# wmtlab/tactileSR

Hardware: AMD Instinct MI355X
Metric: SR samples/sec (4x4->40x40) (higher is better)
Workload: dtype f32 as 2 power-of-two-scaled fp16 planes x 3 MFMA products, fp32 accumulate (fp32-grade); 1 GPU; tactileSR_model eval forward 4x4->40x40, batch=4096/GPU, fp32 in/out (BASELINE configs[1]); batch_per_gpu=4096, scale_factor=10, seqsCnt=1, parallelism=replicas x1, conv_impl=fp16x3, dist_world_size=1

## Files before the change

### tactilesr_amd/csrc/conv_mfma_k32.hip

```cpp
#include "tsr_common.h"
#include "conv_args.h"
#include "conv_epilogue16.h"
#include "conv_fuse1x1_16.h"
#include "tactilesr_hip.h"
#include <type_traits>

typedef _Float16 kf16x8 __attribute__((ext_vector_type(8)));
typedef _Float16 kf16x4 __attribute__((ext_vector_type(4)));

constexpr int k32_row_slots(int px) {
  int rs = px * 4;
  while ((rs & 3) != 2) ++rs;
  return rs;
}

template <int KS, int COUT, int WN, bool DBH = false, int NTHR = 256> struct K32Geom {
  static constexpr int IMG = (NTHR / 64) / WN;
  static constexpr int HH = 8 + KS - 1;
  static constexpr int T = KS * KS;
  static constexpr int HS = (T - 1) / 2;
  static constexpr int PIXB = 64;
  static constexpr int ROWB = k32_row_slots(HH) * 16;
  static constexpr int IMGB = HH * ROWB;
  static constexpr int HALO_B = IMG * IMGB;
  static constexpr int SROWB = k32_row_slots(8) * 16;
  static constexpr int SIMGB = 8 * SROWB;
  static constexpr int SIDE_B = DBH ? 0 : IMG * SIMGB;
  static constexpr int WTAP_B = 2 * 16 * COUT * 2;
  static constexpr int WSLAB_B = 2 * WTAP_B;
  static constexpr int NHB = DBH ? 2 : 1;
  static constexpr int MAIN_LDS = NHB * HALO_B + SIDE_B + 3 * WSLAB_B;
};

constexpr int PAIR_KH[12] = {0, 0, 0, 2, 1, 3, 4, 4, 1, 1, 2, 3};
constexpr int PAIR_KW[12] = {0, 2, 4, 4, 0, 0, 1, 3, 1, 3, 1, 1};
constexpr int PAIR_V[12] = {0, 0, 1, 1, 1, 1, 0, 0, 0, 1, 0, 0};
constexpr int PAIR_OUTER = 8;

template <int KS, int COUT, bool EXT, int WN, bool FUSE2 = false, bool DBH = false, int NTHR = 256, bool PAIR = false>
__global__ __launch_bounds__(NTHR, NTHR == 512 ? 1 : 2) void conv_k32_kernel(const ConvArgs a) {
  static_assert(!PAIR || (KS == 5 && COUT == 128 && !EXT && !FUSE2 && !DBH), "pair form: 5x5 geometry, inference");
  static_assert(COUT == 64 * WN, "every wave owns 64 channels");
  static_assert(!FUSE2 || (!EXT && COUT == 128), "fused 1x1: 128 channels, inference");
  static_assert(NTHR == 256 || (NTHR == 512 && WN == 2), "512 threads: 4 images x 2 C_out halves");
  typedef K32Geom<KS, COUT, WN, DBH, NTHR> G;
  constexpr int NW = NTHR / 64;
  constexpr bool WDMA = !EXT;
  constexpr int IMG = G::IMG, P = KS / 2, HH = G::HH, T = G::T, HS = G::HS, NT = COUT / (16 * WN);
  constexpr int PIXB = G::PIXB, ROWB = G::ROWB, IMGB = G::IMGB, HALO_B = G::HALO_B;
  constexpr int SROWB = G::SROWB, SIMGB = G::SIMGB, SIDE_B = G::SIDE_B;
  constexpr int WTAP_B = G::WTAP_B, WSLAB_B = G::WSLAB_B;
  constexpr int WITEMS = WSLAB_B / 16, WV = (WITEMS + NTHR - 1) / NTHR;
  constexpr int NITEM = IMG * HH * HH * 4, NIT = (NITEM + NTHR - 1) / NTHR;
  constexpr int FUSE_LDS = FUSE2 ? Fuse1x1Geom16<IMG>::BYTES + 64 : 0;
  __shared__ __attribute__((aligned(16))) char lds[G::MAIN_LDS > FUSE_LDS ? G::MAIN_LDS : FUSE_LDS];
  char* halo = lds;
  char* wbuf = lds + G::NHB * HALO_B + SIDE_B;

  const int tid = threadIdx.x;
  const int lane = tid & 63;
  const int wave = tid >> 6;
  const int wave_s = __builtin_amdgcn_readfirstlane(wave);
  const int wm = WN == 2 ? wave >> 1 : wave, wn = WN == 2 ? wave & 1 : 0;
  const int m = lane & 15, g = lane >> 4, khalf = g & 1, tsel = g >> 1;

  float sx = 1.f, accmul = 1.f, sxh = 1.f;
  int bid;
  {
    const int nwg = gridDim.x, q = nwg >> 3, r = nwg & 7;
    const int xcd = blockIdx.x & 7, idx = blockIdx.x >> 3;
    bid = (xcd < r ? xcd * (q + 1) : r * (q + 1) + (xcd - r) * q) + idx;
  }
  const int tpi = a.tiles_x * a.tiles_y;
  const int ig = bid / tpi;
  const int trem = bid - ig * tpi;
  const int ebase = bid * IMG;
  const int ty = trem / a.tiles_x, tx = trem - ty * a.tiles_x;
  const int y0 = ty * 8, x0 = tx * 8, b0 = ig * IMG;
  const int HW = a.H * a.W;
  const int in_blocks = a.in_ctot >> 4;

  int st_src[NIT], st_dst[NIT];
#pragma unroll
  for (int k = 0; k < NIT; ++k) {
    const int it = tid + k * NTHR;
    st_src[k] = -1;
    st_dst[k] = -1;
    if (it < NITEM) {
      const int qd = it & 3, px = it >> 2;
      const int img = px / (HH * HH), rem = px - img * (HH * HH);
      const int hy = rem / HH, hx = rem - hy * HH;
      const int gy = y0 - P + hy, gx = x0 - P + hx, b = b0 + img;
      st_dst[k] = img * IMGB + hy * ROWB + hx * PIXB + qd * 8;
      if (b < a.B && gy >= 0 && gy < a.H && gx >= 0 && gx < a.W)
        st_src[k] = ((img * in_blocks) * HW + gy * a.W + gx) * 16 + qd * 4;
    }
  }
  const float* in_base = a.in + ((size_t)b0 * in_blocks + (a.in_coff >> 4)) * HW * 16;

  const int laneA0 = wm * IMGB + (m >> 3) * ROWB + (m & 7) * PIXB + khalf * 16;
  const int lx = laneA0 + tsel * PIXB;
  constexpr int CK = PAIR ? 3 : KS - 1;
  const int lw = PAIR ? laneA0 + tsel * ROWB
                      : laneA0 + tsel * (ROWB - (KS - 1) * PIXB);
  const int lc = tsel ? laneA0 + CK * ROWB + CK * PIXB
                      : HALO_B + wm * SIMGB + (m >> 3) * SROWB + (m & 7) * PIXB + khalf * 16;
  const int lcs = tsel ? 2 * ROWB : 2 * SROWB;
  const int lcd = laneA0 + (KS - 1) * (ROWB + PIXB) + tsel * HALO_B;
  const int laneB = tsel * WTAP_B + (khalf * COUT + wn * (COUT / WN) + m) * 16;
  const int laneBh = tsel * (WTAP_B / 2) + (khalf * 64 + wn * 32 + m) * 16;

  f32x4 acc[4][NT];
#pragma unroll
  for (int mt = 0; mt < 4; ++mt)
#pragma unroll
    for (int nt = 0; nt < NT; ++nt) acc[mt][nt] = (f32x4){0.f, 0.f, 0.f, 0.f};

  const int nreal = a.cin >> 4;
  const int nchunk = nreal + (nreal & 1);
  const int S = (nchunk >> 1) * T;
  const char* wsrc = (const char*)a.wp;
  const __amdgpu_buffer_rsrc_t wrsrc = __builtin_amdgcn_make_buffer_rsrc((void*)a.wp, 0, 0x7fffffff, 0x00020000);

  f32x4 hsc = {1.f, 1.f, 1.f, 1.f}, hsh = {0.f, 0.f, 0.f, 0.f};
  auto load_halo = [&](int c, f32x4* hv) __attribute__((always_inline)) {
    const float* inc = in_base + (size_t)(c < nreal ? c : nreal - 1) * HW * 16;
    if (EXT && a.in_scale) {
      const int cq = (c < nreal ? c : nreal - 1) * 16 + (tid & 3) * 4;
      hsc = *(const f32x4*)(a.in_scale + cq);
      hsh = *(const f32x4*)(a.in_shift + cq);
    }
#pragma unroll
    for (int k = 0; k < NIT; ++k) hv[k] = *(const f32x4*)(inc + (unsigned)(st_src[k] < 0 ? 0 : st_src[k]));
  };
  auto store_halo = [&](const f32x4* hv, int c, int hb = 0) __attribute__((always_inline)) {
#pragma unroll
    for (int k = 0; k < NIT; ++k) {
      if (st_dst[k] >= 0) {
        f32x4 v = hv[k];
        if (EXT && a.in_scale) {
#pragma unroll
          for (int jj = 0; jj < 4; ++jj) v[jj] = tsr_relu_x2(fmaf(v[jj], hsc[jj], hsh[jj]));
        }
        const bool inside = st_src[k] >= 0 && c < nreal;
#pragma unroll
        for (int jj = 0; jj < 4; ++jj) v[jj] = inside ? v[jj] * sxh : 0.f;
#pragma unroll
        for (int p = 0; p < 2; ++p) {
          kf16x4 bq;
#pragma unroll
          for (int jj = 0; jj < 4; ++jj) {
            bq[jj] = (_Float16)v[jj];
            v[jj] -= (float)bq[jj];
          }
          *(kf16x4*)(halo + hb * HALO_B + st_dst[k] + p * 32) = bq;
        }
      }
    }
  };
#define DMA_BYTES(goff_, slot_, nv_)                                                     \
  {                                                                                      \
    const int vo_ = (int)(goff_) + tid * 16;                                             \
    char* dst_ = wbuf + (slot_) * WSLAB_B + wave_s * 1024;                               \
    _Pragma("unroll") for (int v = 0; v < (nv_); ++v)                                    \
      __builtin_amdgcn_raw_ptr_buffer_load_lds(wrsrc, (__attribute__((address_space(3))) void*)(dst_ + v * NTHR * 16), 16, \
                                               vo_ + v * NTHR * 16, 0, 0, 0);             \
  }
#define LOAD_W(sidx)                                                                     \
  {                                                                                      \
    const f32x4* src_ = (const f32x4*)(wsrc + (size_t)(sidx) * WSLAB_B);                  \
    _Pragma("unroll") for (int v = 0; v < WV; ++v) wreg[v] = src_[tid + v * NTHR];        \
  }
#define STORE_W(slot)                                                                    \
  {                                                                                      \
    char* wb_ = wbuf + (slot) * WSLAB_B;                                                 \
    _Pragma("unroll") for (int v = 0; v < WV; ++v) ((f32x4*)wb_)[tid + v * NTHR] = wreg[v]; \
  }
#define DMA_W(sidx, slot) DMA_BYTES((size_t)(sidx) * WSLAB_B, slot, WV)
#define DMA_WAIT_N(n_) __builtin_amdgcn_s_waitcnt(0x0F70 | ((n_) & 15) | (((n_) >> 4) << 14))
#define DMA_WAIT() DMA_WAIT_N(0)
#define PAIR_HALF(pq_) ((pq_) < 24 && ((pq_) % 12) < PAIR_OUTER)
#define DMA_WP(slot, pq_)                                                                \
  {                                                                                      \
    if (PAIR_HALF(pq_)) { DMA_BYTES(woff, slot, WV / 2); woff += WSLAB_B / 2; }          \
    else { DMA_BYTES(woff, slot, WV); woff += WSLAB_B; }                                 \
  }
#define STEP_BARRIER() __syncthreads()
#define LOAD_A(dst, p_, st_, hb_)                                                        \
  {                                                                                      \
    const int kh_ = PAIR ? PAIR_KH[(st_)] : (2 * (st_)) / KS, kw_ = PAIR ? PAIR_KW[(st_)] : (2 * (st_)) - kh_ * KS; \
    const bool x_ = PAIR ? PAIR_V[(st_)] == 0 : kw_ < KS - 1;                            \
    const char* ab_ = lds + (x_ ? lx : lw) + (hb_) * HALO_B + kh_ * ROWB + kw_ * PIXB + (p_) * 32; \
    _Pragma("unroll") for (int mt = 0; mt < 4; ++mt) dst[mt] = *(const kf16x8*)(ab_ + mt * 2 * ROWB); \
  }
#define LOAD_A_CROSS(dst, p_)                                                            \
  {                                                                                      \
    _Pragma("unroll") for (int mt = 0; mt < 4; ++mt) dst[mt] = *(const kf16x8*)(lds + lc + mt * lcs + (p_) * 32); \
  }
#define LOAD_A_CROSSD(dst, p_)                                                           \
  {                                                                                      \
    _Pragma("unroll") for (int mt = 0; mt < 4; ++mt) dst[mt] = *(const kf16x8*)(lds + lcd + mt * 2 * ROWB + (p_) * 32); \
  }
#define LOAD_B(dst, p_, slot_)                                                           \
  {                                                                                      \
    const char* wb_ = wbuf + (slot_) * WSLAB_B + laneB + (p_) * (2 * COUT * 16);         \
    _Pragma("unroll") for (int nt = 0; nt < NT; ++nt) dst[nt] = *(const kf16x8*)(wb_ + nt * 256); \
  }
#define LOAD_B_HI(dst, p_, slot_)                                                        \
  {                                                                                      \
    const char* wb_ = wbuf + (slot_) * WSLAB_B + laneBh + (p_) * (2 * 64 * 16);          \
    _Pragma("unroll") for (int nt = 2; nt < NT; ++nt) dst[nt] = *(const kf16x8*)(wb_ + (nt - 2) * 256); \
  }
#define MFMA_PHASE_HI(A_, B_)                                                            \
  _Pragma("unroll") for (int mt = 0; mt < 4; ++mt)                                       \
    _Pragma("unroll") for (int nt = 2; nt < NT; ++nt)                                    \
      acc[mt][nt] = __builtin_amdgcn_mfma_f32_16x16x32_f16(A_[mt], B_[nt], acc[mt][nt], 0, 0, 0);
#define MFMA_PHASE(A_, B_)                                                               \
  _Pragma("unroll") for (int mt = 0; mt < 4; ++mt)                                       \
    _Pragma("unroll") for (int nt = 0; nt < NT; ++nt)                                    \
      acc[mt][nt] = __builtin_amdgcn_mfma_f32_16x16x32_f16(A_[mt], B_[nt], acc[mt][nt], 0, 0, 0);
#define INTERLEAVE(n_, per_)                                                             \
  _Pragma("unroll") for (int i_ = 0; i_ < (n_); ++i_) {                                  \
    __builtin_amdgcn_sched_group_barrier(0x008, (per_), 0);                              \
    __builtin_amdgcn_sched_group_barrier(0x100, 1, 0);                                   \
  }

  auto operand_scales = [&]() __attribute__((always_inline)) {
    float mx = a.in_amax ? *a.in_amax : 0.f;
    if (EXT && a.in_scale) {
      __shared__ float bnd[2 * NW];
      float ms = 0.f, mt = 0.f;
      for (int c = threadIdx.x; c < a.cin; c += NTHR) {
        ms = fmaxf(ms, fabsf(a.in_scale[c]));
        mt = fmaxf(mt, fabsf(a.in_shift[c]));
      }
#pragma unroll
      for (int o = 32; o > 0; o >>= 1) {
        ms = fmaxf(ms, __shfl_xor(ms, o));
        mt = fmaxf(mt, __shfl_xor(mt, o));
      }
      if (lane == 0) { bnd[wave * 2] = ms; bnd[wave * 2 + 1] = mt; }
      __syncthreads();
      ms = 0.f; mt = 0.f;
#pragma unroll
      for (int w = 0; w < NW; ++w) { ms = fmaxf(ms, bnd[2 * w]); mt = fmaxf(mt, bnd[2 * w + 1]); }
      mx = mx * ms + mt;
    }
    if (mx > 0.f) {
      int e = (int)((__float_as_uint(mx) >> 23) & 0xFF) - 127;
      int be = 13 - e + 127;
      be = be < 1 ? 1 : (be > 254 ? 254 : be);
      sx = __uint_as_float((unsigned)be << 23);
    }
    float w_inv = a.w_inv_scale;
    if (a.w_amax) {
      const float wmx = *a.w_amax;
      w_inv = 1.f;
      if (wmx > 0.f && wmx < 3.0e38f) {
        int be = 127 - (13 - ((int)((__float_as_uint(wmx) >> 23) & 0xFF) - 127));
        be = be < 1 ? 1 : (be > 254 ? 254 : be);
        w_inv = __uint_as_float((unsigned)be << 23);
      }
    }
    accmul = w_inv / sx;
    sxh = (EXT && a.in_scale) ? 0.5f * sx : sx;
  };

  f32x4 hv[NIT], wreg[WDMA ? 1 : WV];
  size_t woff = 0;
  load_halo(0, hv);
  if constexpr (PAIR) {
    DMA_WP(0, 0);
    DMA_WP(1, 1);
    operand_scales();
  } else if constexpr (WDMA) {
    DMA_W(0, 0);
    if (S > 1) DMA_W(1, 1);
    operand_scales();
  } else {
    LOAD_W(0);
    operand_scales();
    STORE_W(0);
    if (S > 1) { LOAD_W(1); STORE_W(1); }
  }
  store_halo(hv, 0);
  if constexpr (WDMA) { DMA_WAIT(); } else { if (S > 2) LOAD_W(2); }
  __syncthreads();

  kf16x8 A0[4], A1[4], B0[NT] = {}, B1[NT] = {};
  LOAD_A(A1, 1, 0, 0);
  if constexpr (PAIR) { LOAD_B_HI(B0, 0, 0); } else { LOAD_B(B0, 0, 0); }

  constexpr int SCI = IMG * 256 / NTHR, SCS = NTHR / 256;
  const int sc_t = tid & 255, sc_i0 = tid >> 8;
  const int sc_src = sc_i0 * IMGB + ((sc_t >> 5) + CK) * ROWB + (((sc_t >> 2) & 7) + CK) * PIXB + (sc_t & 3) * 16;
  const int sc_dst = HALO_B + sc_i0 * SIMGB + (sc_t >> 5) * SROWB + ((sc_t >> 2) & 7) * PIXB + (sc_t & 3) * 16;

  int s = 0;
  int slot = 0;
  auto block = [&](int c, auto oddc) __attribute__((always_inline)) {
    constexpr int ODD = decltype(oddc)::value;
    constexpr int NST = HS + ODD;
#pragma unroll
    for (int st = 0; st < NST; ++st) {
      const int slot1 = slot == 2 ? 0 : slot + 1;
      const int slot2 = slot1 == 2 ? 0 : slot1 + 1;
      const bool cross = ODD && st == HS;
      f32x4 sidev[SCI];
      if (WDMA && s + 2 < S) {
        if constexpr (PAIR) { DMA_WP(slot2, (ODD * HS + st + 2) % 25); } else { DMA_W(s + 2, slot2); }
      }
      const bool outer = PAIR && st < PAIR_OUTER;
      const bool next_outer = PAIR && (st + 1 < PAIR_OUTER || st + 1 == NST);
      if (cross) { LOAD_A_CROSS(A0, 0); } else { LOAD_A(A0, 0, st, 0); }
      if (outer) { LOAD_B_HI(B1, 1, slot); } else { LOAD_B(B1, 1, slot); }
      if (!ODD && st == 0) {
#pragma unroll
        for (int k = 0; k < SCI; ++k) sidev[k] = *(const f32x4*)(lds + sc_src + k * SCS * IMGB);
      }
      if (st == NST - 2 && c + 1 < nchunk) load_halo(c + 1, hv);
      if (outer) {
        MFMA_PHASE_HI(A1, B0);
        if (!ODD && st == 0) { INTERLEAVE(6 + SCI, 1); } else { INTERLEAVE(6, 1); }
      } else {
        MFMA_PHASE(A1, B0);
        if (!ODD && st == 0) { INTERLEAVE(8 + SCI, 1); } else { INTERLEAVE(8, 2); }
      }
      if (st + 1 < NST) {
        if (ODD && st + 1 == HS) { LOAD_A_CROSS(A1, 1); } else { LOAD_A(A1, 1, st + 1, 0); }
      }
      if (outer) {
        MFMA_PHASE_HI(A0, B0);
        if (st + 1 < NST) { INTERLEAVE(4, 2); }
      } else {
        MFMA_PHASE(A0, B0);
        if (st + 1 < NST) { INTERLEAVE(4, 4); }
      }
      if (next_outer) { LOAD_B_HI(B0, 0, slot1); } else { LOAD_B(B0, 0, slot1); }
      if (outer) {
        MFMA_PHASE_HI(A0, B1);
        if (next_outer) { INTERLEAVE(2, 4); } else { INTERLEAVE(4, 2); }
      } else {
        MFMA_PHASE(A0, B1);
        if (next_outer) { INTERLEAVE(2, 8); } else { INTERLEAVE(4, 4); }
      }
      if (!ODD && st == 0) {
#pragma unroll
        for (int k = 0; k < SCI; ++k) *(f32x4*)(lds + sc_dst + k * SCS * SIMGB) = sidev[k];
      }
      if constexpr (WDMA) {
        if (st == NST - 2 && c + 1 < nchunk) { DMA_WAIT_N(NIT); } else { DMA_WAIT(); }
      } else {
        if (s + 2 < S) STORE_W(slot2);
        if (s + 3 < S) LOAD_W(s + 3);
      }
      STEP_BARRIER();
      if (st + 1 == NST && c + 1 < nchunk) {
        store_halo(hv, c + 1);
        __syncthreads();
        LOAD_A(A1, 1, 0, 0);
      }
      ++s;
      slot = slot1;
    }
  };
  if constexpr (!DBH) {
    for (int c = 0; c < nchunk; c += 2) {
      block(c, std::integral_constant<int, 0>());
      block(c + 1, std::integral_constant<int, 1>());
    }
  } else {
    for (int c = 0; c < nchunk; c += 2) {
#pragma unroll
      for (int p = 0; p < T; ++p) {
        const int slot1 = slot == 2 ? 0 : slot + 1;
        const int slot2 = slot1 == 2 ? 0 : slot1 + 1;
        if (WDMA && s + 2 < S) DMA_W(s + 2, slot2);
        if (p == HS) { LOAD_A_CROSSD(A0, 0); }
        else if (p < HS) { LOAD_A(A0, 0, p, 0); }
        else { LOAD_A(A0, 0, p - HS - 1, 1); }
        LOAD_B(B1, 1, slot);
        if (p == 0) load_halo(c + 1, hv);
        if (p == HS + 1 && c + 2 < nchunk) load_halo(c + 2, hv);
        MFMA_PHASE(A1, B0);
        INTERLEAVE(8, 2);
        if (p + 1 == HS) { LOAD_A_CROSSD(A1, 1); }
        else if (p + 1 < HS) { LOAD_A(A1, 1, p + 1, 0); }
        else if (p + 1 < T) { LOAD_A(A1, 1, p - HS, 1); }
        else { LOAD_A(A1, 1, 0, 0); }
        MFMA_PHASE(A0, B0);
        INTERLEAVE(4, 4);
        LOAD_B(B0, 0, slot1);
        MFMA_PHASE(A0, B1);
        INTERLEAVE(4, 4);
        if (p == HS - 2) store_halo(hv, c + 1, 1);
        if (p == T - 2 && c + 2 < nchunk) store_halo(hv, c + 2, 0);
        if constexpr (WDMA) {
          if (p == 0 || (p == HS + 1 && c + 2 < nchunk)) { DMA_WAIT_N(NIT); } else { DMA_WAIT(); }
        } else {
          if (s + 2 < S) STORE_W(slot2);
          if (s + 3 < S) LOAD_W(s + 3);
        }
        STEP_BARRIER();
        ++s;
        slot = slot1;
      }
    }
  }
#undef DMA_W
#undef LOAD_W
#undef STORE_W
#undef DMA_WP
#undef DMA_BYTES
#undef DMA_WAIT
#undef DMA_WAIT_N
#undef PAIR_HALF
#undef STEP_BARRIER
#undef LOAD_A
#undef LOAD_A_CROSS
#undef LOAD_A_CROSSD
#undef LOAD_B
#undef LOAD_B_HI
#undef MFMA_PHASE_HI
#undef MFMA_PHASE
#undef INTERLEAVE

  if constexpr (FUSE2) conv_fuse1x1_epilogue16<IMG>(a, acc, lds, b0, y0, x0, wm, wn, lane, HW, accmul);
  else conv_epilogue16<COUT, EXT, WN>(a, acc, ebase, b0, y0, x0, wm, wn, lane, HW, accmul);
}

int tsr_conv_k32_images(int cout) { (void)cout; return 4; }

template <int KS, int COUT, bool EXT>
static int launch_k32(const ConvArgs& a, hipStream_t st) {
  constexpr int WN = COUT / 64;
  if constexpr (COUT == 128 && EXT) {
    const int grid = ((a.B + 3) / 4) * a.tiles_x * a.tiles_y;
    hipLaunchKernelGGL((conv_k32_kernel<KS, COUT, EXT, WN, false, KS == 3, 512>), dim3(grid), dim3(512), 0, st, a);
    return tsr_check_launch();
  }
  constexpr int IMG = 4 / WN;
  const int grid = ((a.B + IMG - 1) / IMG) * a.tiles_x * a.tiles_y;
  hipLaunchKernelGGL((conv_k32_kernel<KS, COUT, EXT, WN, false, KS == 3>), dim3(grid), dim3(256), 0, st, a);
  return tsr_check_launch();
}

int tsr_conv_k32(const ConvArgs& a, int cout, int ks, bool ext, hipStream_t st) {
  if (ext) {
    if (cout == 64 && ks == 3) return launch_k32<3, 64, true>(a, st);
    if (cout == 64 && ks == 5) return launch_k32<5, 64, true>(a, st);
    if (cout == 128 && ks == 3) return launch_k32<3, 128, true>(a, st);
    if (cout == 128 && ks == 5) return launch_k32<5, 128, true>(a, st);
  } else {
    if (cout == 64 && ks == 3) return launch_k32<3, 64, false>(a, st);
    if (cout == 64 && ks == 5) return launch_k32<5, 64, false>(a, st);
    if (cout == 128 && ks == 3) return launch_k32<3, 128, false>(a, st);
    if (cout == 128 && ks == 5) return launch_k32<5, 128, false>(a, st);
  }
  return TSR_ERR_ARG;
}

__host__ __device__ inline int pair_logical_channel(int k) {
  const int wn = k >> 6, nt = (k >> 4) & 3, c = k & 15;
  return (nt < 2 ? 0 : 64) + wn * 32 + (nt & 1) * 16 + c;
}
extern "C" int tsr_pair_channel_perm(int* perm128) {
  if (!perm128) return TSR_ERR_ARG;
  for (int k = 0; k < 128; ++k) perm128[k] = pair_logical_channel(k);
  return TSR_OK;
}

__global__ void pack_pair_kernel(const float* __restrict__ w3, const float* __restrict__ w5, _Float16* __restrict__ wp,
                                 int cin, float wscale, const float* __restrict__ w_amax) {
  if (w_amax) {
    const float wm = *w_amax;
    wscale = 1.f;
    if (wm > 0.f && wm < 3.0e38f) {
      int be = 127 + 13 - ((int)((__float_as_uint(wm) >> 23) & 0xFF) - 127);
      be = be < 1 ? 1 : (be > 254 ? 254 : be);
      wscale = __uint_as_float((unsigned)be << 23);
    }
  }
  const int cin_p = (cin + 31) & ~31;
  const size_t total = (size_t)128 * cin_p * 25;
  for (size_t i = blockIdx.x * (size_t)blockDim.x + threadIdx.x; i < total; i += (size_t)gridDim.x * blockDim.x) {
    const int j = i & 7;
    size_t r = i >> 3;
    const int k = r & 127; r >>= 7;
    const int kh2 = r & 1; r >>= 1;
    const int tap = r % 25;
    const int chunk = r / 25;
    const int ci = chunk * 16 + kh2 * 8 + j;
    const int kh = tap / 5, kw = tap - kh * 5;
    const int nt = (k >> 4) & 3, ch = (k >> 6) * 32 + (nt & 1) * 16 + (k & 15);
    float v = 0.f;
    if (ci < cin) {
      if (nt >= 2) v = w5[((size_t)ch * cin + ci) * 25 + tap];
      else if (kh >= 1 && kh <= 3 && kw >= 1 && kw <= 3) v = w3[((size_t)ch * cin + ci) * 9 + (kh - 1) * 3 + (kw - 1)];
    }
    v *= wscale;
    int pos = 24;
#pragma unroll
    for (int st = 0; st < 12; ++st) {
      if (kh == PAIR_KH[st] && kw == PAIR_KW[st]) pos = 2 * st;
      if (kh == PAIR_KH[st] + PAIR_V[st] && kw == PAIR_KW[st] + 1 - PAIR_V[st]) pos = 2 * st + 1;
    }
    const int odd = chunk & 1;
    const bool half = pos < 2 * PAIR_OUTER;
    if (half && nt < 2) continue;
    size_t base = (size_t)(chunk >> 1) * (2 * 65536 + 8192);
    if (pos >= 24) base += 2 * 65536 + (size_t)odd * 4096;
    else if (half) base += (size_t)odd * 65536 + (size_t)(pos >> 1) * 4096 + (size_t)(pos & 1) * 2048;
    else base += (size_t)odd * 65536 + 32768 + (size_t)((pos - 16) >> 1) * 8192 + (size_t)(pos & 1) * 4096;
    const int nch = half ? 64 : 128;
    const int kk = half ? (k >> 6) * 32 + (nt - 2) * 16 + (k & 15) : k;
    for (int p = 0; p < 2; ++p) {
      const _Float16 q = (_Float16)v;
      v -= (float)q;
      wp[base + ((size_t)(p * 2 + kh2) * nch + kk) * 8 + j] = q;
    }
  }
}

extern "C" long long tsr_conv_weight_pair_elems(int cin) { return (long long)(((cin + 31) & ~31) / 32) * (2 * 65536 + 8192); }

extern "C" int tsr_pack_conv_weight_pair_f16s(const float* w3_oihw, const float* w5_oihw, void* w_packed, int cin,
                                              float wscale, const float* w_amax, void* stream) {
  if (!w3_oihw || !w5_oihw || !w_packed || cin <= 0 || (cin & 15) || (!w_amax && !(wscale > 0.f))) return TSR_ERR_ARG;
  const size_t total = (size_t)128 * ((cin + 31) & ~31) * 25;
  const int grid = (int)((total + 255) / 256);
  hipLaunchKernelGGL(pack_pair_kernel, dim3(grid > 4096 ? 4096 : grid), dim3(256), 0, (hipStream_t)stream, w3_oihw,
                     w5_oihw, (_Float16*)w_packed, cin, wscale, w_amax);
  return tsr_check_launch();
}

extern "C" int tsr_conv2d_fwd_f16s_pair(const float* in, int in_ctot, int in_coff, int cin, const void* w_packed,
                                        float w_inv_scale, const float* in_amax, float* out_amax,
                                        const float* scale, const float* shift, float* out, int out_ctot, int out_coff,
                                        int relu, int B, int H, int W, void* stream) {
  if (!in || !w_packed || !out || !in_amax || B <= 0 || H <= 0 || W <= 0 || !(w_inv_scale > 0.f)) return TSR_ERR_ARG;
  if ((cin & 15) || (in_ctot & 15) || (in_coff & 15) || (out_ctot & 15) || (out_coff & 15) || cin <= 0 ||
      in_coff + cin > in_ctot || out_coff + 128 > out_ctot)
    return TSR_ERR_ARG;
  ConvArgs a = {};
  a.in = in; a.in_ctot = in_ctot; a.in_coff = in_coff; a.cin = cin;
  a.wp = (const float*)w_packed; a.scale = scale; a.shift = shift;
  a.out = out; a.out_ctot = out_ctot; a.out_coff = out_coff; a.relu = relu;
  a.B = B; a.H = H; a.W = W;
  a.tiles_x = (W + 7) / 8; a.tiles_y = (H + 7) / 8;
  a.in_amax = in_amax; a.w_inv_scale = w_inv_scale; a.out_amax = out_amax;
  const int grid = ((B + 1) / 2) * a.tiles_x * a.tiles_y;
  hipLaunchKernelGGL((conv_k32_kernel<5, 128, false, 2, false, false, 256, true>), dim3(grid), dim3(256), 0,
                     (hipStream_t)stream, a);
  return tsr_check_launch();
}

int tsr_conv_k32_fuse1x1(const ConvArgs& a, int ks, hipStream_t st) {
  const int grid = ((a.B + 1) / 2) * a.tiles_x * a.tiles_y;
  if (ks == 5) hipLaunchKernelGGL((conv_k32_kernel<5, 128, false, 2, true>), dim3(grid), dim3(256), 0, st, a);
  else hipLaunchKernelGGL((conv_k32_kernel<3, 128, false, 2, true, true>), dim3(grid), dim3(256), 0, st, a);
  return tsr_check_launch();
}
```

Baseline: 32490 samples/s.

## Use double-buffered halo and two-slab plane-ring weight DMA for 5x5 128-channel conv

For the 5x5, 128-channel inference conv (plain and fused-1x1), the kernel now uses a double-buffered halo instead of the side buffer. To fit LDS, the three-slot weight ring becomes a two-slab ring. Weights are streamed per tap-plane with buffer-to-LDS DMA, in a reordered slab sequence that matches the cross-chunk halo schedule. The goal is more overlap of halo and weight loads with MFMA work, at the cost of tighter DMA/barrier ordering and a risk of hazards on the shortened weight ring.

Measured after the change: 32750 samples/s (median of 6 runs). No clear change (+0.8%).

```diff
diff --git a/tactilesr_amd/csrc/conv_mfma_k32.hip b/tactilesr_amd/csrc/conv_mfma_k32.hip
--- a/tactilesr_amd/csrc/conv_mfma_k32.hip
+++ b/tactilesr_amd/csrc/conv_mfma_k32.hip
@@ -29,7 +29,8 @@
   static constexpr int WTAP_B = 2 * 16 * COUT * 2;
   static constexpr int WSLAB_B = 2 * WTAP_B;
   static constexpr int NHB = DBH ? 2 : 1;
-  static constexpr int MAIN_LDS = NHB * HALO_B + SIDE_B + 3 * WSLAB_B;
+  static constexpr bool PRING = DBH && KS == 5;
+  static constexpr int MAIN_LDS = NHB * HALO_B + SIDE_B + (PRING ? 2 : 3) * WSLAB_B;
 };
 
 constexpr int PAIR_KH[12] = {0, 0, 0, 2, 1, 3, 4, 4, 1, 1, 2, 3};
@@ -43,9 +44,11 @@
   static_assert(COUT == 64 * WN, "every wave owns 64 channels");
   static_assert(!FUSE2 || (!EXT && COUT == 128), "fused 1x1: 128 channels, inference");
   static_assert(NTHR == 256 || (NTHR == 512 && WN == 2), "512 threads: 4 images x 2 C_out halves");
+  static_assert(!(DBH && KS == 5) || (COUT == 128 && !EXT && NTHR == 256), "5x5 double-buffered halo: 128 channels, inference");
   typedef K32Geom<KS, COUT, WN, DBH, NTHR> G;
   constexpr int NW = NTHR / 64;
   constexpr bool WDMA = !EXT;
+  constexpr bool PRING = G::PRING;
   constexpr int IMG = G::IMG, P = KS / 2, HH = G::HH, T = G::T, HS = G::HS, NT = COUT / (16 * WN);
   constexpr int PIXB = G::PIXB, ROWB = G::ROWB, IMGB = G::IMGB, HALO_B = G::HALO_B;
   constexpr int SROWB = G::SROWB, SIMGB = G::SIMGB, SIDE_B = G::SIDE_B;
@@ -108,6 +111,7 @@
   const int lcs = tsel ? 2 * ROWB : 2 * SROWB;
   const int lcd = laneA0 + (KS - 1) * (ROWB + PIXB) + tsel * HALO_B;
   const int laneB = tsel * WTAP_B + (khalf * COUT + wn * (COUT / WN) + m) * 16;
+  const int laneBp = tsel * (WTAP_B / 2) + (khalf * COUT + wn * (COUT / WN) + m) * 16;
   const int laneBh = tsel * (WTAP_B / 2) + (khalf * 64 + wn * 32 + m) * 16;
 
   f32x4 acc[4][NT];
@@ -184,6 +188,19 @@
   {                                                                                      \
     if (PAIR_HALF(pq_)) { DMA_BYTES(woff, slot, WV / 2); woff += WSLAB_B / 2; }          \
     else { DMA_BYTES(woff, slot, WV); woff += WSLAB_B; }                                 \
+  }
+#define SLAB_OF(q_) ((q_) < HS ? (q_) : (q_) == HS ? T - 1 : (q_) - 1)
+#define DMA_PLANE(sg_, pl_, so_)                                                         \
+  {                                                                                      \
+    _Pragma("unroll") for (int t_ = 0; t_ < 2; ++t_)                                     \
+      __builtin_amdgcn_raw_ptr_buffer_load_lds(                                          \
+          wrsrc, (__attribute__((address_space(3))) void*)(wbuf + (so_) + (pl_) * WTAP_B + t_ * (WTAP_B / 2) + wave_s * 1024), \
+          16, tid * 16, wbase + (sg_) * WSLAB_B + t_ * WTAP_B + (pl_) * (WTAP_B / 2), 0, 0); \
+  }
+#define LOAD_BP(dst, off_)                                                               \
+  {                                                                                      \
+    const char* wb_ = wbuf + (off_) + laneBp;                                            \
+    _Pragma("unroll") for (int nt = 0; nt < NT; ++nt) dst[nt] = *(const kf16x8*)(wb_ + nt * 256); \
   }
 #define STEP_BARRIER() __syncthreads()
 #define LOAD_A(dst, p_, st_, hb_)                                                        \
@@ -268,8 +285,14 @@
 
   f32x4 hv[NIT], wreg[WDMA ? 1 : WV];
   size_t woff = 0;
+  int wbase = 0;
   load_halo(0, hv);
-  if constexpr (PAIR) {
+  if constexpr (PRING) {
+    DMA_PLANE(0, 0, 0);
+    DMA_PLANE(0, 1, 0);
+    DMA_PLANE(1, 0, WSLAB_B);
+    operand_scales();
+  } else if constexpr (PAIR) {
     DMA_WP(0, 0);
     DMA_WP(1, 1);
     operand_scales();
@@ -289,7 +312,7 @@
 
   kf16x8 A0[4], A1[4], B0[NT] = {}, B1[NT] = {};
   LOAD_A(A1, 1, 0, 0);
-  if constexpr (PAIR) { LOAD_B_HI(B0, 0, 0); } else { LOAD_B(B0, 0, 0); }
+  if constexpr (PRING) { LOAD_BP(B0, 0); } else if constexpr (PAIR) { LOAD_B_HI(B0, 0, 0); } else { LOAD_B(B0, 0, 0); }
 
   constexpr int SCI = IMG * 256 / NTHR, SCS = NTHR / 256;
   const int sc_t = tid & 255, sc_i0 = tid >> 8;
@@ -370,16 +393,20 @@
       block(c + 1, std::integral_constant<int, 1>());
     }
   } else {
+    int wpo = 0, wpn = WSLAB_B;
     for (int c = 0; c < nchunk; c += 2) {
 #pragma unroll
       for (int p = 0; p < T; ++p) {
         const int slot1 = slot == 2 ? 0 : slot + 1;
         const int slot2 = slot1 == 2 ? 0 : slot1 + 1;
-        if (WDMA && s + 2 < S) DMA_W(s + 2, slot2);
+        if constexpr (PRING) {
+          if (s + 1 < S) DMA_PLANE(p + 1 < T ? SLAB_OF(p + 1) : T + SLAB_OF(p + 1 - T), 1, wpn);
+          if (s + 2 < S) DMA_PLANE(p + 2 < T ? SLAB_OF(p + 2) : T + SLAB_OF(p + 2 - T), 0, wpo);
+        } else if (WDMA && s + 2 < S) DMA_W(s + 2, slot2);
         if (p == HS) { LOAD_A_CROSSD(A0, 0); }
         else if (p < HS) { LOAD_A(A0, 0, p, 0); }
         else { LOAD_A(A0, 0, p - HS - 1, 1); }
-        LOAD_B(B1, 1, slot);
+        if constexpr (PRING) { LOAD_BP(B1, wpo + WTAP_B); } else { LOAD_B(B1, 1, slot); }
         if (p == 0) load_halo(c + 1, hv);
         if (p == HS + 1 && c + 2 < nchunk) load_halo(c + 2, hv);
         MFMA_PHASE(A1, B0);
@@ -390,7 +417,7 @@
         else { LOAD_A(A1, 1, 0, 0); }
         MFMA_PHASE(A0, B0);
         INTERLEAVE(4, 4);
-        LOAD_B(B0, 0, slot1);
+        if constexpr (PRING) { LOAD_BP(B0, wpn); } else { LOAD_B(B0, 0, slot1); }
         MFMA_PHASE(A0, B1);
         INTERLEAVE(4, 4);
         if (p == HS - 2) store_halo(hv, c + 1, 1);
@@ -404,13 +431,19 @@
         STEP_BARRIER();
         ++s;
         slot = slot1;
-      }
+        wpo = wpn;
+        wpn = WSLAB_B - wpo;
+      }
+      wbase += T * WSLAB_B;
     }
   }
 #undef DMA_W
 #undef LOAD_W
 #undef STORE_W
 #undef DMA_WP
+#undef DMA_PLANE
+#undef LOAD_BP
+#undef SLAB_OF
 #undef DMA_BYTES
 #undef DMA_WAIT
 #undef DMA_WAIT_N
@@ -441,7 +474,7 @@
   }
   constexpr int IMG = 4 / WN;
   const int grid = ((a.B + IMG - 1) / IMG) * a.tiles_x * a.tiles_y;
-  hipLaunchKernelGGL((conv_k32_kernel<KS, COUT, EXT, WN, false, KS == 3>), dim3(grid), dim3(256), 0, st, a);
+  hipLaunchKernelGGL((conv_k32_kernel<KS, COUT, EXT, WN, false, KS == 3 || (COUT == 128 && !EXT)>), dim3(grid), dim3(256), 0, st, a);
   return tsr_check_launch();
 }
 
@@ -557,7 +590,7 @@
 
 int tsr_conv_k32_fuse1x1(const ConvArgs& a, int ks, hipStream_t st) {
   const int grid = ((a.B + 1) / 2) * a.tiles_x * a.tiles_y;
-  if (ks == 5) hipLaunchKernelGGL((conv_k32_kernel<5, 128, false, 2, true>), dim3(grid), dim3(256), 0, st, a);
+  if (ks == 5) hipLaunchKernelGGL((conv_k32_kernel<5, 128, false, 2, true, true>), dim3(grid), dim3(256), 0, st, a);
   else hipLaunchKernelGGL((conv_k32_kernel<3, 128, false, 2, true, true>), dim3(grid), dim3(256), 0, st, a);
   return tsr_check_launch();
 }
```
